# zuds-survey/zuds-pipeline

Hardware: AMD Instinct MI355X
Metric: Mpix/s resample->coadd->subtract, 3072x3072 frames (higher is better)
Workload: dtype f32; 1 GPU; configs[1]+[2]: 32x 3072x3072 TPV frames/GPU, mesh background + weight rescale + Lanczos-3 resample + WEIGHTED coadd (+ AND mask coadd, int16 masks); then 1 science frame/GPU: align ref, hotpants 3x3 regions x 10x10 stamps, r=10, ko=4, subtract; frames_per_gpu=32, size=3072, mask_dtype=int16, combine=WEIGHTED, subtract=True

## Files before the change

zuds-pipeline_amd/csrc/hp_apply.hip:

```cpp
#include "hp_dev.h"

__device__ inline double xs_bg(const double* __restrict__ xsol, int reg, const hp_plan& P, int t) {
    return xsol[(size_t)reg * P.nunk + 1 + (size_t)(P.nc - 1) * P.nkp + t];
}

constexpr int apply_bank_passes(int pitch, int lpr, int r, int step) {
    int worst = 0;
    for (int half = 0; half < 2; ++half) {
        int cnt[64] = {};
        for (int l = 32 * half; l < 32 * half + 32; ++l) {
            const int row = l / lpr, strip = l % lpr;
            if (row >= step) continue;
            const int e = row * pitch + strip * r;
            ++cnt[(2 * e) % 64];
            ++cnt[(2 * e + 1) % 64];
        }
        for (int b = 0; b < 64; ++b) worst = cnt[b] > worst ? cnt[b] : worst;
    }
    return worst;
}
constexpr int apply_pitch(int width, int lpr, int r, int step) {
    int best = width, bw = apply_bank_passes(width, lpr, r, step);
    for (int p = width + 1; p <= width + 16; ++p) {
        const int w = apply_bank_passes(p, lpr, r, step);
        if (w < bw) { bw = w; best = p; }
    }
    return best;
}

constexpr int apply_pitch_n(int width, int lpr, int r, int step, int range) {
    int best = width, bw = apply_bank_passes(width, lpr, r, step);
    for (int p = width + 1; p <= width + range; ++p) {
        const int w = apply_bank_passes(p, lpr, r, step);
        if (w < bw) { bw = w; best = p; }
    }
    return best;
}

template <int HWK> struct apply_cfg {
    enum { STEP = 2 * HWK + 1,
           LPR = (STEP <= 11) ? 1 : (STEP <= 22 ? 2 : 3),
           R = (STEP + LPR - 1) / LPR,
           LPB = STEP * LPR,
           NB = 256 / LPB > 0 ? 256 / LPB : 1,
           TW = NB * STEP + 2 * HWK,
           TP = apply_pitch(NB * STEP + 2 * HWK, LPR, (STEP + LPR - 1) / LPR, STEP) };
};

template <int HWK>
__global__ __launch_bounds__(256) void k_hp_apply(const hp_plan P, const unsigned long long* __restrict__ solved_mask,
                                                  const float* __restrict__ sci,
                                                  const float* __restrict__ ref,
                                                  const float* __restrict__ srms,
                                                  const float* __restrict__ trms,
                                                  const uint8_t* __restrict__ outbad,
                                                  const double* __restrict__ filt,
                                                  const double* __restrict__ xsol,
                                                  float* __restrict__ diff,
                                                  float* __restrict__ noise,
                                                  int* __restrict__ nmasked) {
    const int reg = blockIdx.z;
    const int solved = (int)((*solved_mask >> reg) & 1ull);
    typedef apply_cfg<HWK> C;
    constexpr int STEP = C::STEP, R = C::R, LPR = C::LPR, LPB = C::LPB, NB = C::NB;
    constexpr int TW = C::TW;
    constexpr int TP = C::TP;
    constexpr int TH = STEP + 2 * HWK;
    typedef float ap_v2f __attribute__((ext_vector_type(2)));
    extern __shared__ float ap_smem[];
    ap_v2f* tTV = reinterpret_cast<ap_v2f*>(ap_smem);
    const int tvn = max(TH * TP, P.nunk + 2 * P.nc + (NB + 1) * P.nf1 * STEP + NB + 2 * NB * P.nkp);
    ap_v2f* kc = tTV + tvn;
    double* cf = reinterpret_cast<double*>(kc + NB * STEP * STEP);
    __shared__ int wmask[4];
    double* xs = reinterpret_cast<double*>(ap_smem);
    double* ts = xs + P.nunk;
    double* sb = ts + P.nc;
    double* fl = sb + P.nc;
    double* gf = fl + P.nf1 * STEP;
    double* s0v = gf + NB * P.nf1 * STEP;
    double* pxy = s0v + NB;
    const int tid = threadIdx.x;
    const int x0r = P.rx0[reg], x1r = P.rx1[reg], y0r = P.ry0[reg], y1r = P.ry1[reg];
    const int gx0 = x0r + blockIdx.x * NB * STEP;
    const int gy0 = y0r + blockIdx.y * STEP;
    if (gx0 >= x1r || gy0 >= y1r) return;
    const double xc = x0r + 0.5 * (x1r - x0r), hx = 0.5 * (x1r - x0r);
    const double yc = y0r + 0.5 * (y1r - y0r), hy = 0.5 * (y1r - y0r);
    const double* x = xsol + (size_t)reg * P.nunk;
    for (int e0 = tid; e0 < P.nunk; e0 += 256 * 4) {
        double t[4];
#pragma unroll
        for (int u = 0; u < 4; ++u) t[u] = (e0 + 256 * u < P.nunk) ? x[e0 + 256 * u] : 0.0;
#pragma unroll
        for (int u = 0; u < 4; ++u)
            if (e0 + 256 * u < P.nunk) xs[e0 + 256 * u] = t[u];
    }
    for (int e0 = tid; e0 < P.nf1 * STEP; e0 += 256 * 4) {
        double t[4];
#pragma unroll
        for (int u = 0; u < 4; ++u) t[u] = (e0 + 256 * u < P.nf1 * STEP) ? filt[e0 + 256 * u] : 0.0;
#pragma unroll
        for (int u = 0; u < 4; ++u)
            if (e0 + 256 * u < P.nf1 * STEP) fl[e0 + 256 * u] = t[u];
    }
    for (int e = tid; e < P.nc; e += 256) { ts[e] = P.tscale[e]; sb[e] = P.tsub0[e] ? 1.0 : 0.0; }
    for (int e = tid; e < NB * P.nkp; e += 256) {
        const int b = e / P.nkp, pp = e - b * P.nkp;
        const double fx = (gx0 + b * STEP + HWK - xc) / hx, fy = (gy0 + HWK - yc) / hy;
        pxy[2 * e] = ipowd(fx, P.kpi[pp]);
        pxy[2 * e + 1] = ipowd(fy, P.kpj[pp]);
    }
    __syncthreads();
    for (int e = tid; e < NB * P.nc; e += 256) {
        int b = e / P.nc, n = e - b * P.nc;
        double v;
        if (n == 0) v = xs[0];
        else {
            v = 0.0;
            const double* xb = xs + 1 + (n - 1) * P.nkp;
            const double* pb = pxy + 2 * b * P.nkp;
            for (int p = 0; p < P.nkp; ++p) v += xb[p] * pb[2 * p] * pb[2 * p + 1];
        }
        cf[e] = v;
    }
    __syncthreads();
    if (tid < NB) {
        double t = 0.0;
        for (int n = 0; n < P.nc; ++n) t += cf[tid * P.nc + n] * sb[n];
        s0v[tid] = t;
    }
    __syncthreads();
    for (int e = tid; e < NB * STEP * P.ngauss; e += 256) {
        const int g = e / (NB * STEP), r = e - g * NB * STEP;
        const int b = r / STEP, v = r - b * STEP;
        const double* cb = cf + b * P.nc;
        const int deg = P.gdeg[g], fb = P.gbase[g];
        int n = P.gterm0[g];
        for (int a = 0; a <= deg; ++a) {
            double acc = 0.0;
            for (int bb = 0; bb <= deg - a; ++bb, ++n) acc += cb[n] * ts[n] * fl[(fb + bb) * STEP + v];
            if (fb + a == P.tfx[0])
                acc -= s0v[b] * ts[0] * fl[P.tfy[0] * STEP + v];
            gf[((size_t)b * P.nf1 + fb + a) * STEP + v] = acc;
        }
    }
    __syncthreads();
    for (int e = tid; e < NB * STEP * STEP; e += 256) {
        const int b = e / (STEP * STEP), tap = e - b * STEP * STEP;
        const int v = tap / STEP, u = tap - v * STEP;
        const double* gb = gf + (size_t)b * P.nf1 * STEP + v;
        double acc = 0.0;
#pragma unroll 5
        for (int f = 0; f < P.nf1; ++f) acc += fl[f * STEP + u] * gb[f * STEP];
        const float k = (float)acc;
        kc[e] = (ap_v2f){k, k * k};
    }
    const double bg0 = xs[1 + (size_t)(P.nc - 1) * P.nkp];
    const float norm = P.normalize ? (float)(1.0 / xs[0]) : 1.f;
    __syncthreads();
    {
        constexpr int NIT = (TH * TW + 255) / 256;
        float tt[NIT], tr[NIT];
#pragma unroll
        for (int it = 0; it < NIT; ++it) {
            const int e = tid + 256 * it;
            const int yy = e / TW, xx = e - yy * TW;
            const int gx = gx0 - HWK + xx, gy = gy0 - HWK + yy;
            tt[it] = 0.f;
            tr[it] = 0.f;
            if (e < TH * TW && gx >= 0 && gx < P.nx && gy >= 0 && gy < P.ny) {
                const size_t idx = (size_t)gy * P.nx + gx;
                tt[it] = ref[idx];
                tr[it] = trms[idx];
            }
        }
#pragma unroll
        for (int it = 0; it < NIT; ++it) {
            const int e = tid + 256 * it;
            float t = tt[it], v = tr[it] * tr[it];
            if (!(fabsf(t) < 3e38f)) t = 0.f;
            if (!(fabsf(v) < 3e38f)) v = 0.f;
            if (e < TH * TW) tTV[(e / TW) * TP + e % TW] = (ap_v2f){t, v};
        }
    }
    __syncthreads();
    const int b = tid / LPB;
    const int l = tid - b * LPB;
    const int row = l / LPR, strip = l - row * LPR;
    const int ox0 = b * STEP + strip * R;
    const bool live = b < NB && gy0 + row < y1r && gy0 + row < P.ny;
    ap_v2f acc2[R];
#pragma unroll
    for (int q = 0; q < R; ++q) acc2[q] = (ap_v2f){0.f, 0.f};
    if (live) {
        const ap_v2f* kb = kc + b * STEP * STEP;
        for (int v = -HWK; v <= HWK; ++v) {
            const ap_v2f* rt = tTV + (row + HWK - v) * TP + ox0;
            ap_v2f w2[R + 2 * HWK];
#pragma unroll
            for (int q = 0; q < R + 2 * HWK; ++q) w2[q] = rt[q];
            const ap_v2f* kr = kb + (v + HWK) * STEP;
#pragma unroll
            for (int u = -HWK; u <= HWK; ++u) {
                const ap_v2f k2 = kr[u + HWK];
#pragma unroll
                for (int q = 0; q < R; ++q) acc2[q] = __builtin_elementwise_fma(k2, w2[q + HWK - u], acc2[q]);
            }
        }
    }
    constexpr int OW = NB * STEP;
    __syncthreads();
    if (live) {
#pragma unroll
        for (int q = 0; q < R; ++q)
            if (strip * R + q < STEP) tTV[row * OW + ox0 + q] = acc2[q];
    }
    __syncthreads();
    int masked = 0;
    {
        constexpr int NE = (STEP * OW + 255) / 256;
        float es[NE], er[NE];
        bool eb[NE], ein[NE];
#pragma unroll
        for (int it = 0; it < NE; ++it) {
            const int e = tid + 256 * it;
            const int orow = e / OW, ocol = e - orow * OW;
            const int gx = gx0 + ocol, gy = gy0 + orow;
            ein[it] = e < STEP * OW && gx < x1r && gx < P.nx && gy < y1r && gy < P.ny;
            es[it] = er[it] = 0.f;
            eb[it] = true;
            if (ein[it]) {
                const size_t idx = (size_t)gy * P.nx + gx;
                eb[it] = outbad[idx] != 0;
                es[it] = sci[idx];
                er[it] = srms[idx];
            }
        }
#pragma unroll
        for (int it = 0; it < NE; ++it) {
            if (!ein[it]) continue;
            const int e = tid + 256 * it;
            const int orow = e / OW, ocol = e - orow * OW;
            const int gx = gx0 + ocol, gy = gy0 + orow;
            const size_t idx = (size_t)gy * P.nx + gx;
            float d = P.fi, nz = P.fin;
            if (solved && !eb[it]) {
                double bg = bg0;
                if (P.nbg > 1) {
                    const double xf = (gx - xc) / hx, yf = (gy - yc) / hy;
                    bg = 0.0;
                    for (int t = 0; t < P.nbg; ++t)
                        bg += xs_bg(xsol, reg, P, t) * ipowd(xf, P.bpi[t]) * ipowd(yf, P.bpj[t]);
                }
                const ap_v2f a = tTV[e];
                d = (es[it] - a.x - (float)bg) * norm;
                nz = sqrtf(fmaxf(er[it] * er[it] + a.y, 0.f)) * fabsf(norm);
            } else {
                masked += 1;
            }
            diff[idx] = d;
            noise[idx] = nz;
        }
    }
#pragma unroll
    for (int o = 32; o >= 1; o >>= 1) masked += __shfl_xor(masked, o);
    if ((tid & 63) == 0) wmask[tid >> 6] = masked;
    __syncthreads();
    if (tid == 0) {
        const int tot = wmask[0] + wmask[1] + wmask[2] + wmask[3];
        if (tot) atomicAdd(nmasked, tot);
    }
}

template <int HWK> struct applyw_cfg {
    enum { STEP = 2 * HWK + 1,
           LPR = 64 / STEP > 0 ? 64 / STEP : 1,
           R = (STEP + LPR - 1) / LPR,
           NBW = 4,
           TW = NBW * STEP + 2 * HWK,
           TH = STEP + 2 * HWK,
           TP = apply_pitch_n(NBW * STEP + 2 * HWK, 64 / STEP > 0 ? 64 / STEP : 1,
                              (STEP + (64 / STEP > 0 ? 64 / STEP : 1) - 1) / (64 / STEP > 0 ? 64 / STEP : 1), STEP, 32) };
    enum { EFF = (100 * STEP * LPR / 64) * STEP / (LPR * R) };
};

#define HPK_MAXP 15
#define HPK_NBK 16
template <int HWK>
__global__ __launch_bounds__(256) void k_hp_kbasis(const hp_plan P, const double* __restrict__ filt,
                                                   const double* __restrict__ xsol, double* __restrict__ Mt) {
    constexpr int STEP = 2 * HWK + 1, NT = STEP * STEP;
    const int reg = blockIdx.y, p = blockIdx.x;
    const double* x = xsol + (size_t)reg * P.nunk;
    __shared__ double xq[HP_MAXX], sn[HP_MAXX], flt[HP_MAXF1 * STEP];
    __shared__ int txn[HP_MAXX], tyn[HP_MAXX], sbn[HP_MAXX];
    const int tid = threadIdx.x;
    for (int n = tid; n < P.nc; n += 256) {
        sn[n] = P.tscale[n];
        txn[n] = P.tfx[n] * STEP;
        tyn[n] = P.tfy[n] * STEP;
        sbn[n] = P.tsub0[n];
        xq[n] = (n >= 1 && p < P.nkp) ? x[1 + (size_t)(n - 1) * P.nkp + p] : 0.0;
    }
    for (int e = tid; e < P.nf1 * STEP; e += 256) flt[e] = filt[e];
    __syncthreads();
    for (int tap = tid; tap < NT; tap += 256) {
        const int v = tap / STEP, u = tap - v * STEP;
        const double b0 = sn[0] * flt[tyn[0] + v] * flt[txn[0] + u];
        double acc = 0.0;
        if (p == HPK_MAXP) {
            acc = x[0] * (b0 - (sbn[0] ? b0 : 0.0));
        } else if (p < P.nkp) {
#pragma unroll 8
            for (int n = 1; n < P.nc; ++n) {
                const double bn = sn[n] * flt[tyn[n] + v] * flt[txn[n] + u];
                acc += xq[n] * (bn - (sbn[n] ? b0 : 0.0));
            }
        }
        Mt[((size_t)reg * (HPK_MAXP + 1) + p) * NT + tap] = acc;
    }
}

template <int HWK>
__global__ __launch_bounds__(512) void k_hp_ktable(const hp_plan P, const double* __restrict__ Mt, int maxbx, int maxby,
                                                   float2* __restrict__ kcg) {
    constexpr int STEP = 2 * HWK + 1, NT = STEP * STEP, TPT = (NT + 511) / 512;
    __shared__ double W[HPK_NBK][HPK_MAXP + 1];
    const int reg = blockIdx.z, tid = threadIdx.x;
    const int x0r = P.rx0[reg], x1r = P.rx1[reg], y0r = P.ry0[reg], y1r = P.ry1[reg];
    const int bx0 = blockIdx.x * HPK_NBK;
    const int gx0 = x0r + bx0 * STEP, gy0 = y0r + blockIdx.y * STEP;
    if (gx0 >= x1r || gy0 >= y1r) return;
    const double xc = x0r + 0.5 * (x1r - x0r), hx = 0.5 * (x1r - x0r);
    const double yc = y0r + 0.5 * (y1r - y0r), hy = 0.5 * (y1r - y0r);
    for (int e = tid; e < HPK_NBK * (HPK_MAXP + 1); e += 512) {
        const int b = e / (HPK_MAXP + 1), pp = e - b * (HPK_MAXP + 1);
        double w = 0.0;
        if (pp < P.nkp) {
            const double fx = (gx0 + b * STEP + HWK - xc) / hx, fy = (gy0 + HWK - yc) / hy;
            w = ipowd(fx, P.kpi[pp]) * ipowd(fy, P.kpj[pp]);
        }
        W[b][pp] = w;
    }
    double m[TPT][HPK_MAXP + 1];
#pragma unroll
    for (int t = 0; t < TPT; ++t)
#pragma unroll
        for (int pp = 0; pp <= HPK_MAXP; ++pp) {
            const int tap = min(tid + 512 * t, NT - 1);
            m[t][pp] = Mt[((size_t)reg * (HPK_MAXP + 1) + pp) * NT + tap];
        }
    __syncthreads();
    for (int b = 0; b < HPK_NBK; ++b) {
        const int bx = bx0 + b;
        if (bx >= maxbx || gx0 + b * STEP >= x1r) break;
        float2* out = kcg + (((size_t)reg * maxby + blockIdx.y) * maxbx + bx) * NT;
        double w[HPK_MAXP];
#pragma unroll
        for (int pp = 0; pp < HPK_MAXP; ++pp) w[pp] = W[b][pp];
#pragma unroll
        for (int t = 0; t < TPT; ++t) {
            double acc = m[t][HPK_MAXP];
#pragma unroll
            for (int pp = 0; pp < HPK_MAXP; ++pp) acc = fma(w[pp], m[t][pp], acc);
            const float k = (float)acc;
            const int tap = tid + 512 * t;
            if (tap < NT) out[tap] = make_float2(k, k * k);
        }
    }
}

template <int HWK>
__global__ __launch_bounds__(256) void k_hp_apply_w(const hp_plan P, const unsigned long long* __restrict__ solved_mask,
                                                    const float* __restrict__ sci,
                                                    const float* __restrict__ ref,
                                                    const float* __restrict__ srms,
                                                    const float* __restrict__ trms,
                                                    const uint8_t* __restrict__ outbad,
                                                    const double* __restrict__ xsol,
                                                    const float2* __restrict__ kcg, int maxbx, int maxby,
                                                    float* __restrict__ diff,
                                                    float* __restrict__ noise,
                                                    int* __restrict__ nmasked) {
    const int reg = blockIdx.z;
    const int solved = (int)((*solved_mask >> reg) & 1ull);
    typedef applyw_cfg<HWK> C;
    constexpr int STEP = C::STEP, R = C::R, LPR = C::LPR, NB = C::NBW, TW = C::TW, TP = C::TP, TH = C::TH;
    typedef float ap_v2f __attribute__((ext_vector_type(2)));
    extern __shared__ float apw_smem[];
    ap_v2f* tTV = reinterpret_cast<ap_v2f*>(apw_smem);
    __shared__ int wmask[4];
    const int tid = threadIdx.x;
    const int x0r = P.rx0[reg], x1r = P.rx1[reg], y0r = P.ry0[reg], y1r = P.ry1[reg];
    const int gx0 = x0r + blockIdx.x * NB * STEP;
    const int gy0 = y0r + blockIdx.y * STEP;
    if (gx0 >= x1r || gy0 >= y1r) return;
    const double xc = x0r + 0.5 * (x1r - x0r), hx = 0.5 * (x1r - x0r);
    const double yc = y0r + 0.5 * (y1r - y0r), hy = 0.5 * (y1r - y0r);
    const double bg0 = xsol[(size_t)reg * P.nunk + 1 + (size_t)(P.nc - 1) * P.nkp];
    const float norm = P.normalize ? (float)(1.0 / xsol[(size_t)reg * P.nunk]) : 1.f;
    {
        constexpr int NIT = (TH * TW + 255) / 256;
        float tt[NIT], tr[NIT];
#pragma unroll
        for (int it = 0; it < NIT; ++it) {
            const int e = tid + 256 * it;
            const int yy = e / TW, xx = e - yy * TW;
            const int gx = gx0 - HWK + xx, gy = gy0 - HWK + yy;
            tt[it] = 0.f;
            tr[it] = 0.f;
            if (e < TH * TW && gx >= 0 && gx < P.nx && gy >= 0 && gy < P.ny) {
                const size_t idx = (size_t)gy * P.nx + gx;
                tt[it] = ref[idx];
                tr[it] = trms[idx];
            }
        }
#pragma unroll
        for (int it = 0; it < NIT; ++it) {
            const int e = tid + 256 * it;
            float t = tt[it], v = tr[it] * tr[it];
            if (!(fabsf(t) < 3e38f)) t = 0.f;
            if (!(fabsf(v) < 3e38f)) v = 0.f;
            if (e < TH * TW) tTV[(e / TW) * TP + e % TW] = (ap_v2f){t, v};
        }
    }
    __syncthreads();
    const int b = __builtin_amdgcn_readfirstlane(tid >> 6);
    const int l = tid & 63;
    const int row = l / LPR, strip = l - row * LPR;
    const int ox0 = b * STEP + strip * R;
    const bool live = row < STEP && gx0 + b * STEP < x1r && gy0 + row < y1r && gy0 + row < P.ny;
    ap_v2f acc2[R];
#pragma unroll
    for (int q = 0; q < R; ++q) acc2[q] = (ap_v2f){0.f, 0.f};
    {
        const int bxi = min((int)blockIdx.x * NB + b, maxbx - 1);
        const ap_v2f* kb = reinterpret_cast<const ap_v2f*>(kcg) +
                           (((size_t)reg * maxby + blockIdx.y) * maxbx + bxi) * (STEP * STEP);
        const int rowc = min(row, STEP - 1);
#pragma unroll 1
        for (int v = -HWK; v <= HWK; ++v) {
            const ap_v2f* rt = tTV + (rowc + HWK - v) * TP + ox0;
            ap_v2f w2[R + 2 * HWK];
#pragma unroll
            for (int q = 0; q < R + 2 * HWK; ++q) w2[q] = rt[(LPR * R == STEP) ? q : min(q, TW - 1 - ox0)];
            const ap_v2f* kr = kb + (v + HWK) * STEP;
#pragma unroll
            for (int u = -HWK; u <= HWK; ++u) {
                const ap_v2f k2 = kr[u + HWK];
#pragma unroll
                for (int q = 0; q < R; ++q) acc2[q] = __builtin_elementwise_fma(k2, w2[q + HWK - u], acc2[q]);
            }
        }
    }
    constexpr int OW = NB * STEP;
    __syncthreads();
    if (live) {
#pragma unroll
        for (int q = 0; q < R; ++q)
            if (strip * R + q < STEP) tTV[row * OW + ox0 + q] = acc2[q];
    }
    __syncthreads();
    int masked = 0;
    {
        constexpr int NE = (STEP * OW + 255) / 256;
        float es[NE], er[NE];
        bool eb[NE], ein[NE];
#pragma unroll
        for (int it = 0; it < NE; ++it) {
            const int e = tid + 256 * it;
            const int orow = e / OW, ocol = e - orow * OW;
            const int gx = gx0 + ocol, gy = gy0 + orow;
            ein[it] = e < STEP * OW && gx < x1r && gx < P.nx && gy < y1r && gy < P.ny;
            es[it] = er[it] = 0.f;
            eb[it] = true;
            if (ein[it]) {
                const size_t idx = (size_t)gy * P.nx + gx;
                eb[it] = outbad[idx] != 0;
                es[it] = sci[idx];
                er[it] = srms[idx];
            }
        }
#pragma unroll
        for (int it = 0; it < NE; ++it) {
            if (!ein[it]) continue;
            const int e = tid + 256 * it;
            const int orow = e / OW, ocol = e - orow * OW;
            const int gx = gx0 + ocol, gy = gy0 + orow;
            const size_t idx = (size_t)gy * P.nx + gx;
            float d = P.fi, nz = P.fin;
            if (solved && !eb[it]) {
                double bg = bg0;
                if (P.nbg > 1) {
                    const double xf = (gx - xc) / hx, yf = (gy - yc) / hy;
                    bg = 0.0;
                    for (int t = 0; t < P.nbg; ++t)
                        bg += xs_bg(xsol, reg, P, t) * ipowd(xf, P.bpi[t]) * ipowd(yf, P.bpj[t]);
                }
                const ap_v2f a = tTV[e];
                d = (es[it] - a.x - (float)bg) * norm;
                nz = sqrtf(fmaxf(er[it] * er[it] + a.y, 0.f)) * fabsf(norm);
            } else {
                masked += 1;
            }
            diff[idx] = d;
            noise[idx] = nz;
        }
    }
#pragma unroll
    for (int o = 32; o >= 1; o >>= 1) masked += __shfl_xor(masked, o);
    if ((tid & 63) == 0) wmask[tid >> 6] = masked;
    __syncthreads();
    if (tid == 0) {
        const int tot = wmask[0] + wmask[1] + wmask[2] + wmask[3];
        if (tot) atomicAdd(nmasked, tot);
    }
}

template <int HWK>
static int launch_apply(zm_ctx* ctx, const hp_plan& P, const unsigned long long* solved_mask, const float* sci,
                        const float* ref, const float* srms, const float* trms, const uint8_t* outbad,
                        const double* filt, const double* xsol, float* diff, float* noise,
                        int* nmasked) {
    typedef apply_cfg<HWK> C;
    constexpr int STEP = C::STEP, NB = C::NB;
    constexpr int TP = C::TP, TH = STEP + 2 * HWK;
    const size_t tvn = std::max((size_t)TH * TP, (size_t)P.nunk + 2 * (size_t)P.nc + (size_t)(NB + 1) * P.nf1 * STEP + NB + (size_t)2 * NB * P.nkp);
    size_t fl = 2 * tvn + (size_t)2 * NB * STEP * STEP;
    size_t shmem = fl * sizeof(float) + (size_t)NB * P.nc * sizeof(double);
    size_t& set_max = ctx->hp_set_max[HWK];
    if (set_max < 65536) set_max = 65536;
    if (shmem > set_max) {
        ZM_HIP(hipFuncSetAttribute((const void*)k_hp_apply<HWK>,
                                   hipFuncAttributeMaxDynamicSharedMemorySize, (int)shmem));
        set_max = shmem;
    }
    int W = 0, H = 0;
    for (int reg = 0; reg < P.nreg; ++reg) {
        W = std::max(W, P.rx1[reg] - P.rx0[reg]);
        H = std::max(H, P.ry1[reg] - P.ry0[reg]);
    }
    typedef applyw_cfg<HWK> CW;
    const char* form = getenv("ZM_APPLY_FORM");
    const bool wave_form = (form ? !strcmp(form, "wave") : (CW::EFF >= 60 && HWK >= 4)) && P.nkp <= HPK_MAXP;
    if (wave_form && !(form && !strcmp(form, "tile"))) {
        const int maxbx = zm_div_up(W, STEP), maxby = zm_div_up(H, STEP);
        float2* kcg = nullptr;
        ZM_TRY(ctx->get("hp_kcg", sizeof(float2) * (size_t)P.nreg * maxby * maxbx * STEP * STEP, (void**)&kcg));
        double* Mt = nullptr;
        ZM_TRY(ctx->get("hp_kmt", sizeof(double) * (size_t)P.nreg * (HPK_MAXP + 1) * STEP * STEP, (void**)&Mt));
        hipLaunchKernelGGL(k_hp_kbasis<HWK>, dim3(HPK_MAXP + 1, P.nreg), dim3(256), 0, ctx->stream, P, filt, xsol, Mt);
        hipLaunchKernelGGL(k_hp_ktable<HWK>, dim3(zm_div_up(maxbx, HPK_NBK), maxby, P.nreg), dim3(512), 0, ctx->stream,
                           P, Mt, maxbx, maxby, kcg);
        const size_t wsh = sizeof(float2) * (size_t)CW::TH * CW::TP;
        static bool wset[HP_MAX_HWK + 1][64] = {};
        if (wsh > 65536 && !wset[HWK][ctx->device & 63]) {
            ZM_HIP(hipFuncSetAttribute((const void*)k_hp_apply_w<HWK>, hipFuncAttributeMaxDynamicSharedMemorySize, (int)wsh));
            wset[HWK][ctx->device & 63] = true;
        }
        hipLaunchKernelGGL(k_hp_apply_w<HWK>, dim3(zm_div_up(maxbx, CW::NBW), maxby, P.nreg), dim3(256), wsh, ctx->stream,
                           P, solved_mask, sci, ref, srms, trms, outbad, xsol, kcg, maxbx, maxby, diff, noise, nmasked);
        ZM_HIP(hipGetLastError());
        return 0;
    }
    dim3 grd(zm_div_up(zm_div_up(W, STEP), NB), zm_div_up(H, STEP), P.nreg);
    hipLaunchKernelGGL(k_hp_apply<HWK>, grd, dim3(256), shmem, ctx->stream, P, solved_mask, sci, ref, srms,
                       trms, outbad, filt, xsol, diff, noise, nmasked);
    ZM_HIP(hipGetLastError());
    return 0;
}


int zm_hp_launch_apply(zm_ctx* ctx, const hp_plan& P, const unsigned long long* solved_mask, const float* sci,
                       const float* ref, const float* srms, const float* trms, const uint8_t* outbad,
                       const double* filt, const double* xsol, float* diff, float* noise, int* nmasked) {
#define C(H) case H: return launch_apply<H>(ctx, P, solved_mask, sci, ref, srms, trms, outbad, filt, xsol, diff, noise, nmasked);
    switch (P.hwk) {
        C(1) C(2) C(3) C(4) C(5) C(6) C(7) C(8) C(9) C(10) C(11) C(12) C(13) C(14) C(15) C(16) C(17) C(18) C(19) C(20)
        default: zm_set_error("zm_subtract: unsupported kernel half width %d", P.hwk); return 2;
    }
#undef C
}
```

Measured before the change: 50500 Mpix/s.

## Stream kernel taps via scalar loads and inline-asm LDS windows in hotpants apply

```diff
diff --git a/zuds-pipeline_amd/csrc/hp_apply.hip b/zuds-pipeline_amd/csrc/hp_apply.hip
--- a/zuds-pipeline_amd/csrc/hp_apply.hip
+++ b/zuds-pipeline_amd/csrc/hp_apply.hip
@@ -1,4 +1,5 @@
 #include "hp_dev.h"
+#include <utility>
 
 __device__ inline double xs_bg(const double* __restrict__ xsol, int reg, const hp_plan& P, int t) {
     return xsol[(size_t)reg * P.nunk + 1 + (size_t)(P.nc - 1) * P.nkp + t];
@@ -371,6 +372,100 @@
     }
 }
 
+typedef float apw_v2f __attribute__((ext_vector_type(2)));
+typedef float apw_v4f __attribute__((ext_vector_type(4)));
+typedef float apw_v8f __attribute__((ext_vector_type(8)));
+typedef float apw_v16f __attribute__((ext_vector_type(16)));
+
+template <int Q>
+__device__ __forceinline__ void apw_lds_pair(unsigned a, apw_v2f& o) {
+    asm volatile("ds_read_b64 %0, %1 offset:%2" : "=v"(o) : "v"(a), "n"(Q * 8));
+}
+template <int N, int... Q>
+__device__ __forceinline__ void apw_lds_window(unsigned a, apw_v2f (&w)[N], std::integer_sequence<int, Q...>) {
+    (apw_lds_pair<Q>(a, w[Q]), ...);
+}
+
+template <int STEP> struct apw_taps {
+    enum { ND = 2 * STEP, NA = ND / 16,
+           NP = ND <= 58 ? NA : 2,
+           H8 = (ND >> 3) & 1, H4 = (ND >> 2) & 1, H2 = (ND >> 1) & 1,
+           OB = 16 * NA, OC = OB + 8 * H8, OD = OC + 4 * H4, ROWB = 4 * ND };
+    apw_v16f a[NP ? NP : 1];
+    apw_v8f b;
+    apw_v4f c;
+    apw_v2f d;
+    template <int I, int OFF> __device__ __forceinline__ void load(const float* p) {
+        if constexpr (I < NA)
+            asm volatile("s_load_dwordx16 %0, %1, %2" : "=&s"(a[I % (NP ? NP : 1)]) : "s"(p), "n"(OFF + 64 * I));
+        else if constexpr (I == NA && H8) asm volatile("s_load_dwordx8 %0, %1, %2" : "=&s"(b) : "s"(p), "n"(OFF + 4 * OB));
+        else if constexpr (I == NA + 1 && H4) asm volatile("s_load_dwordx4 %0, %1, %2" : "=&s"(c) : "s"(p), "n"(OFF + 4 * OC));
+        else if constexpr (I == NA + 2 && H2) asm volatile("s_load_dwordx2 %0, %1, %2" : "=&s"(d) : "s"(p), "n"(OFF + 4 * OD));
+    }
+    template <int... I> __device__ __forceinline__ void load_first(const float* p, std::integer_sequence<int, I...>) {
+        ((I < NP || I >= NA ? load<I, 0>(p) : (void)0), ...);
+    }
+    static constexpr int last_tap(int i) {
+        return i < NA ? 8 * i + 7 : i == NA ? (H8 ? OB / 2 + 3 : -1) : i == NA + 1 ? (H4 ? OC / 2 + 1 : -1)
+                                  : i == NA + 2 ? (H2 ? OD / 2 : -1) : -1;
+    }
+    static constexpr bool ends_a_piece(int t) {
+        for (int i = 0; i < NA + 3; ++i)
+            if (last_tap(i) == t) return true;
+        return false;
+    }
+    template <int T, int I> __device__ __forceinline__ void after_one(const float* cur) {
+        if constexpr (last_tap(I) == T) {
+            if constexpr (I < NA && I + NP < NA) load<I + NP, 0>(cur);
+            else if constexpr (I < NA) load<I % (NP ? NP : 1), ROWB>(cur);
+            else load<I, ROWB>(cur);
+        }
+    }
+    template <int T, int... I> __device__ __forceinline__ void after(const float* cur, std::integer_sequence<int, I...>) {
+        (after_one<T, I>(cur), ...);
+    }
+    template <int T> __device__ __forceinline__ void before() {
+        if constexpr (T % 8 == 0 && T / 8 < NA && T / 8 >= NP) {
+            asm volatile("s_waitcnt lgkmcnt(0)" ::: "memory");
+            asm volatile("" : "+s"(a[(T / 8) % (NP ? NP : 1)]));
+        }
+    }
+    template <int T> __device__ __forceinline__ apw_v2f tap() const {
+        constexpr int D = 2 * T;
+        if constexpr (D < OB) return (apw_v2f){a[(D / 16) % (NP ? NP : 1)][D % 16], a[(D / 16) % (NP ? NP : 1)][D % 16 + 1]};
+        else if constexpr (H8 && D < OC) return (apw_v2f){b[D - OB], b[D - OB + 1]};
+        else if constexpr (H4 && D < OD) return (apw_v2f){c[D - OC], c[D - OC + 1]};
+        else return d;
+    }
+    __device__ __forceinline__ void pin() {
+#pragma unroll
+        for (int i = 0; i < NP; ++i) asm volatile("" : "+s"(a[i]));
+        if (H8) asm volatile("" : "+s"(b));
+        if (H4) asm volatile("" : "+s"(c));
+        if (H2) asm volatile("" : "+s"(d));
+    }
+};
+
+template <int STEP, int R, int HWK, int U, int NW>
+__device__ __forceinline__ void apw_tap(apw_taps<STEP>& T, const float* cur, const apw_v2f (&w2)[NW], apw_v2f (&acc2)[R]) {
+    T.template before<U>();
+    const apw_v2f k2 = T.template tap<U>();
+#pragma unroll
+    for (int q = 0; q < R; ++q) acc2[q] = __builtin_elementwise_fma(k2, w2[q + 2 * HWK - U], acc2[q]);
+    if constexpr (apw_taps<STEP>::ends_a_piece(U)) {
+#pragma unroll
+        for (int q = 0; q < R; ++q) asm volatile("" : "+v"(acc2[q]));
+        T.template after<U>(cur, std::make_integer_sequence<int, apw_taps<STEP>::NA + 3>());
+#pragma unroll
+        for (int q = 0; q < R; ++q) asm volatile("" : "+v"(acc2[q]));
+    }
+}
+template <int STEP, int R, int HWK, int NW, int... U>
+__device__ __forceinline__ void apw_row(apw_taps<STEP>& T, const float* cur, const apw_v2f (&w2)[NW], apw_v2f (&acc2)[R],
+                                        std::integer_sequence<int, U...>) {
+    (apw_tap<STEP, R, HWK, U>(T, cur, w2, acc2), ...);
+}
+
 template <int HWK>
 __global__ __launch_bounds__(256) void k_hp_apply_w(const hp_plan P, const unsigned long long* __restrict__ solved_mask,
                                                     const float* __restrict__ sci,
@@ -400,7 +495,44 @@
     const double yc = y0r + 0.5 * (y1r - y0r), hy = 0.5 * (y1r - y0r);
     const double bg0 = xsol[(size_t)reg * P.nunk + 1 + (size_t)(P.nc - 1) * P.nkp];
     const float norm = P.normalize ? (float)(1.0 / xsol[(size_t)reg * P.nunk]) : 1.f;
-    {
+    if (gx0 - HWK >= 0 && gx0 - HWK + TW <= P.nx && gy0 - HWK >= 0 && gy0 - HWK + TH <= P.ny) {
+        static_assert(TW % 2 == 0, "the tile is fetched as pairs of columns");
+        typedef float ap_v2u __attribute__((ext_vector_type(2), aligned(4)));
+        constexpr int PW = TW / 2, NP = TH * PW, NIT = (NP + 255) / 256;
+        constexpr int DR = 256 / PW, DC = 256 % PW;
+        const float* r0 = ref + (size_t)(gy0 - HWK) * P.nx + (gx0 - HWK);
+        const float* q0 = trms + (size_t)(gy0 - HWK) * P.nx + (gx0 - HWK);
+        ap_v2u tt[NIT], tr[NIT];
+        int yy = tid / PW, xx = tid - yy * PW;
+        const int yy0 = yy, xx0 = xx;
+#pragma unroll
+        for (int it = 0; it < NIT; ++it) {
+            const bool in = it < NIT - 1 || tid + 256 * it < NP;
+            const size_t o = in ? (size_t)yy * P.nx + 2 * xx : 0;
+            tt[it] = *reinterpret_cast<const ap_v2u*>(r0 + o);
+            tr[it] = *reinterpret_cast<const ap_v2u*>(q0 + o);
+            xx += DC;
+            yy += DR;
+            if (xx >= PW) { xx -= PW; yy += 1; }
+        }
+        yy = yy0;
+        xx = xx0;
+#pragma unroll
+        for (int it = 0; it < NIT; ++it) {
+            float t0 = tt[it].x, v0 = tr[it].x * tr[it].x, t1 = tt[it].y, v1 = tr[it].y * tr[it].y;
+            if (!(fabsf(t0) < 3e38f)) t0 = 0.f;
+            if (!(fabsf(v0) < 3e38f)) v0 = 0.f;
+            if (!(fabsf(t1) < 3e38f)) t1 = 0.f;
+            if (!(fabsf(v1) < 3e38f)) v1 = 0.f;
+            if (it < NIT - 1 || tid + 256 * it < NP) {
+                tTV[yy * TP + 2 * xx] = (ap_v2f){t0, v0};
+                tTV[yy * TP + 2 * xx + 1] = (ap_v2f){t1, v1};
+            }
+            xx += DC;
+            yy += DR;
+            if (xx >= PW) { xx -= PW; yy += 1; }
+        }
+    } else {
         constexpr int NIT = (TH * TW + 255) / 256;
         float tt[NIT], tr[NIT];
 #pragma unroll
@@ -439,20 +571,25 @@
         const ap_v2f* kb = reinterpret_cast<const ap_v2f*>(kcg) +
                            (((size_t)reg * maxby + blockIdx.y) * maxbx + bxi) * (STEP * STEP);
         const int rowc = min(row, STEP - 1);
+        apw_taps<STEP> T;
+        const float* cur = reinterpret_cast<const float*>(kb);
+        unsigned wa = (unsigned)(size_t)(tTV + (rowc + 2 * HWK) * TP + ox0);
+        T.load_first(cur, std::make_integer_sequence<int, apw_taps<STEP>::NA + 3>());
 #pragma unroll 1
-        for (int v = -HWK; v <= HWK; ++v) {
-            const ap_v2f* rt = tTV + (rowc + HWK - v) * TP + ox0;
+        for (int vi = 0; vi < STEP; ++vi) {
             ap_v2f w2[R + 2 * HWK];
-#pragma unroll
-            for (int q = 0; q < R + 2 * HWK; ++q) w2[q] = rt[(LPR * R == STEP) ? q : min(q, TW - 1 - ox0)];
-            const ap_v2f* kr = kb + (v + HWK) * STEP;
-#pragma unroll
-            for (int u = -HWK; u <= HWK; ++u) {
-                const ap_v2f k2 = kr[u + HWK];
-#pragma unroll
-                for (int q = 0; q < R; ++q) acc2[q] = __builtin_elementwise_fma(k2, w2[q + HWK - u], acc2[q]);
-            }
-        }
+            apw_lds_window(wa, w2, std::make_integer_sequence<int, R + 2 * HWK>());
+            asm volatile("s_waitcnt lgkmcnt(0)" ::: "memory");
+            T.pin();
+#pragma unroll
+            for (int q = 0; q < R + 2 * HWK; ++q) asm volatile("" : "+v"(w2[q]));
+            apw_row<STEP, R, HWK>(T, cur, w2, acc2, std::make_integer_sequence<int, STEP>());
+            cur += 2 * STEP;
+            asm volatile("" : "+s"(cur));
+            wa -= TP * 8;
+        }
+        asm volatile("s_waitcnt lgkmcnt(0)" ::: "memory");
+        T.pin();
     }
     constexpr int OW = NB * STEP;
     __syncthreads();
@@ -466,31 +603,36 @@
     {
         constexpr int NE = (STEP * OW + 255) / 256;
         float es[NE], er[NE];
-        bool eb[NE], ein[NE];
+        unsigned ob[NE];
+        bool ein[NE];
+        size_t ei[NE];
+        const size_t idx0 = (size_t)gy0 * P.nx + gx0;
 #pragma unroll
         for (int it = 0; it < NE; ++it) {
             const int e = tid + 256 * it;
             const int orow = e / OW, ocol = e - orow * OW;
             const int gx = gx0 + ocol, gy = gy0 + orow;
             ein[it] = e < STEP * OW && gx < x1r && gx < P.nx && gy < y1r && gy < P.ny;
-            es[it] = er[it] = 0.f;
-            eb[it] = true;
-            if (ein[it]) {
-                const size_t idx = (size_t)gy * P.nx + gx;
-                eb[it] = outbad[idx] != 0;
-                es[it] = sci[idx];
-                er[it] = srms[idx];
-            }
-        }
+            ei[it] = ein[it] ? (size_t)gy * P.nx + gx : idx0;
+        }
+#pragma unroll
+        for (int it = 0; it < NE; ++it) {
+            ob[it] = outbad[ei[it]];
+            es[it] = sci[ei[it]];
+            er[it] = srms[ei[it]];
+        }
+#pragma unroll
+        for (int it = 0; it < NE; ++it) asm volatile("" : "+v"(ob[it]), "+v"(es[it]), "+v"(er[it]));
 #pragma unroll
         for (int it = 0; it < NE; ++it) {
             if (!ein[it]) continue;
             const int e = tid + 256 * it;
             const int orow = e / OW, ocol = e - orow * OW;
             const int gx = gx0 + ocol, gy = gy0 + orow;
-            const size_t idx = (size_t)gy * P.nx + gx;
+            const size_t idx = ei[it];
+            const bool eb = ob[it] != 0;
             float d = P.fi, nz = P.fin;
-            if (solved && !eb[it]) {
+            if (solved && !eb) {
                 double bg = bg0;
                 if (P.nbg > 1) {
                     const double xf = (gx - xc) / hx, yf = (gy - yc) / hy;
@@ -547,13 +689,13 @@
     if (wave_form && !(form && !strcmp(form, "tile"))) {
         const int maxbx = zm_div_up(W, STEP), maxby = zm_div_up(H, STEP);
         float2* kcg = nullptr;
-        ZM_TRY(ctx->get("hp_kcg", sizeof(float2) * (size_t)P.nreg * maxby * maxbx * STEP * STEP, (void**)&kcg));
+        ZM_TRY(ctx->get("hp_kcg", sizeof(float2) * ((size_t)P.nreg * maxby * maxbx * STEP * STEP + STEP), (void**)&kcg));
         double* Mt = nullptr;
         ZM_TRY(ctx->get("hp_kmt", sizeof(double) * (size_t)P.nreg * (HPK_MAXP + 1) * STEP * STEP, (void**)&Mt));
         hipLaunchKernelGGL(k_hp_kbasis<HWK>, dim3(HPK_MAXP + 1, P.nreg), dim3(256), 0, ctx->stream, P, filt, xsol, Mt);
         hipLaunchKernelGGL(k_hp_ktable<HWK>, dim3(zm_div_up(maxbx, HPK_NBK), maxby, P.nreg), dim3(512), 0, ctx->stream,
                            P, Mt, maxbx, maxby, kcg);
-        const size_t wsh = sizeof(float2) * (size_t)CW::TH * CW::TP;
+        const size_t wsh = sizeof(float2) * ((size_t)CW::TH * CW::TP + (CW::LPR * CW::R - CW::STEP));
         static bool wset[HP_MAX_HWK + 1][64] = {};
         if (wsh > 65536 && !wset[HWK][ctx->device & 63]) {
             ZM_HIP(hipFuncSetAttribute((const void*)k_hp_apply_w<HWK>, hipFuncAttributeMaxDynamicSharedMemorySize, (int)wsh));
```

New measurement: 50780 Mpix/s, median of 6. No clear change (+0.6%).
